# Veason-silverbullet/NNR

Measured on AMD Instinct MI355X. Metric: training impressions/sec on MIND-200k (CNE+SUE, bs=64), higher is better.
Workload: dtype f32

## Files before the change

### include/nnr_hip.h

```cpp
#ifndef NNR_HIP_H
#define NNR_HIP_H
#include <stdint.h>
#include <hip/hip_runtime_api.h>

#ifdef __cplusplus
extern "C" {
#endif

#define NNR_OK 0
#define NNR_ERR_ARG (-1)
#define NNR_ERR_LAUNCH (-2)
#define NNR_ERR_UNSUPPORTED (-3)

int nnr_version(void);

typedef struct nnr_gemm_args {
  const float* A;
  const float* B;
  float* C;
  int M, N, K;
  int lda, ldb, ldc;
  int trans_a, trans_b;
  const int* dyn_dev;
  int dyn_dim;
// ... 13 lines not shown
  int ldaux;
  const float* mul;
  int ldmul;
  const float* resid;
  int ldres;
  int accumulate;
  int atomic;
  const int* c_idx;
  int split_k;
  const float* rowdot_w;
  float* rowdot_out;
  int batch;
  long strideA, strideB, strideC, stride_aux, stride_res;
  int k_chunk;
  float* colsum_out;
  int tile;
  uint32_t drop_thresh;
  float drop_scale;
  int vec_epi;
  int sched;
  float* slab;
  long slab_floats;
  int slab_mode;
  const float* pre_add;
  int ldpre;
  int gate_bwd;
  const void* B3;
  long b3_stride;
  int ldb3;
} nnr_gemm_args;

int nnr_gemm_f32(const nnr_gemm_args* args, hipStream_t stream);
int nnr_split_bf16x3(const float* w, int rows, int cols, int ld, int ldo, void* out3, long img_stride, hipStream_t stream);

int nnr_seq_plan(uint8_t* mask, const int* ids, int n, int L, const int* perm_in, int* len_out, int* order, int* rank, int* slen,
                 int* bs, int* off, int* row_seq, int* tok, int* prev_f, int* prev_r, hipStream_t stream);

int nnr_seq_plan_pair(uint8_t* mask0, const int* ids0, int n0, uint8_t* mask1, const int* ids1, int n1, int L, const int* perm_in,
                      int* len_out, int* order, int* rank, int* slen, int* bs, int* off, int* row_seq, int* tok, int* prev_f,
                      int* prev_r, hipStream_t stream);

int nnr_cne_pair_map(const int* order_t, const int* order_c, int n0, int n, int* pm_t, int* pm_c, int* tmp, hipStream_t stream);

int nnr_mask_cover(const uint8_t* mask, int n, int L, uint8_t* cover, hipStream_t stream);
int nnr_seq_rowmap(const int* off, const int* rank, const int* len, int n, int L, int* rowmap, hipStream_t stream);

int nnr_lstm_dims(int H, int* UB, int* HP, int* NP);
int nnr_lstm_pack_weights(const float* w_ih_f, const float* w_hh_f, const float* b_ih_f, const float* b_hh_f, const float* w_ih_r,
                          const float* w_hh_r, const float* b_ih_r, const float* b_hh_r, int H, int E, float* w_ihp, float* b_p,
                          float* wf, float* wb, float* w_ihp_t, hipStream_t stream);
int nnr_lstm_unpack_grads(float* dw_ihp, float* db_p, float* dw_hhp, int H, int E, float* dw_ih_f, float* dw_hh_f,
                          float* db_ih_f, float* db_hh_f, float* dw_ih_r, float* dw_hh_r, float* db_ih_r, float* db_hh_r,
                          int accumulate , int zero_src, hipStream_t stream);
typedef struct nnr_lstm_problem {
  const int* bs; const int* off; const int* slen; const int* prev_f; const int* prev_r;
  int n, L;
  float* gates;
  float* cell;
  float* hout;
  float* cn;
  const float* wf;
  const float* wb;
  const float* dh;
  const float* dcn;
  unsigned* sync;
} nnr_lstm_problem;
// ... 202 lines not shown
```

### nnr_amd/_lib.py

```python
import ctypes as C
import os
import subprocess

_HERE = os.path.dirname(os.path.abspath(__file__))
LIB_PATH = os.environ.get('NNR_HIP_LIB') or os.path.join(_HERE, 'libnnr_hip.so')
_lib = None

vp, ci, cf, cu32, cl = C.c_void_p, C.c_int, C.c_float, C.c_uint32, C.c_long


class GemmArgs(C.Structure):
    _fields_ = [('A', vp), ('B', vp), ('C', vp), ('M', ci), ('N', ci), ('K', ci), ('lda', ci), ('ldb', ci), ('ldc', ci),
                ('trans_a', ci), ('trans_b', ci), ('dyn_dev', vp), ('dyn_dim', ci), ('a_idx', vp), ('b_idx', vp),
                ('drop_target', ci), ('drop_p', cf), ('drop_seed', cu32), ('drop_cols', ci), ('alpha', cf), ('bias', vp),
                ('rowvec', vp), ('ldrv', ci), ('rowvec_map', vp), ('act', ci), ('aux_out', vp), ('ldaux', ci), ('mul', vp),
                ('ldmul', ci), ('resid', vp), ('ldres', ci), ('accumulate', ci), ('atomic', ci), ('c_idx', vp),
                ('split_k', ci), ('rowdot_w', vp), ('rowdot_out', vp), ('batch', ci), ('strideA', cl), ('strideB', cl),
                ('strideC', cl), ('stride_aux', cl), ('stride_res', cl), ('k_chunk', ci), ('colsum_out', vp), ('tile', ci), ('drop_thresh', cu32),
                ('drop_scale', cf), ('vec_epi', ci), ('sched', ci), ('slab', vp), ('slab_floats', cl), ('slab_mode', ci), ('pre_add', vp), ('ldpre', ci), ('gate_bwd', ci), ('B3', vp), ('b3_stride', cl), ('ldb3', ci)]


class LstmProblem(C.Structure):
    _fields_ = [('bs', vp), ('off', vp), ('slen', vp), ('prev_f', vp), ('prev_r', vp), ('n', ci), ('L', ci), ('gates', vp),
                ('cell', vp), ('hout', vp), ('cn', vp), ('wf', vp), ('wb', vp), ('dh', vp), ('dcn', vp), ('sync', vp)]


class TransposeDesc(C.Structure):
    _fields_ = [('inp', vp), ('out', vp), ('rows', ci), ('cols', ci)]


class CorpusTables(C.Structure):
    _fields_ = [(k, vp) for k in ('news_category', 'news_subCategory', 'title_text', 'title_mask', 'title_entity', 'abstract_text',
                                  'abstract_mask', 'abstract_entity', 'beh_user', 'beh_history', 'beh_history_mask', 'beh_line',
                                  'graph_table', 'cmask_table', 'cidx_table')] + [(k, ci) for k in ('T', 'C', 'H', 'G', 'K1')]


class BatchOut(C.Structure):
    _fields_ = [(k, vp) for k in ('user_id', 'u_cat', 'u_sub', 'u_tt', 'u_tm', 'u_te', 'u_ct', 'u_cm', 'u_ce', 'u_hmask', 'u_graph',
                                  'u_cmask', 'u_cidx', 'n_cat', 'n_sub', 'n_tt', 'n_tm', 'n_te', 'n_ct', 'n_cm', 'n_ce')]


class PoolArgs(C.Structure):
    _fields_ = [('x', vp), ('ldx', ci), ('D', ci), ('n', ci), ('L', ci), ('packed', ci), ('off', vp), ('slen', vp),
                ('order', vp), ('mask', vp), ('mask_div', ci), ('score', vp), ('v', vp), ('ldv', ci), ('scale', cf),
                ('alpha', vp), ('out', vp), ('ldo', ci), ('add_in', vp), ('ldadd', ci), ('dout', vp), ('lddo', ci),
                ('dout2', vp), ('lddo2', ci), ('dx', vp), ('lddx', ci), ('dx_accumulate', ci), ('dscore', vp), ('dv', vp),
                ('lddv', ci), ('th', vp), ('ldth', ci), ('A', ci), ('w2', vp),
                ('alpha_b', vp), ('dout_b', vp), ('lddo_b', ci), ('dscore_b', vp), ('v_b', vp), ('ldv_b', ci), ('scale_b', cf)]


SYMBOLS = [
    'nnr_version', 'nnr_gemm_f32', 'nnr_split_bf16x3', 'nnr_seq_plan', 'nnr_seq_plan_pair', 'nnr_cne_pair_map', 'nnr_lstm_dims', 'nnr_lstm_pack_weights', 'nnr_lstm_unpack_grads',
    'nnr_lstm_fwd', 'nnr_lstm_bwd', 'nnr_lstm_sync_bytes', 'nnr_lstm_sync_diag_offset', 'nnr_lstm_set_timeout_counter', 'nnr_attn_pool_fwd', 'nnr_attn_pool_bwd', 'nnr_gate_bwd', 'nnr_packed_seq_sum',
    'nnr_tanh_score_bwd', 'nnr_slot_workspace_floats', 'nnr_colsum', 'nnr_rowdot', 'nnr_small_embed_fwd', 'nnr_small_embed_bwd', 'nnr_add', 'nnr_add_atomic', 'nnr_add2d', 'nnr_expand_rows_fwd', 'nnr_expand_rows_bwd', 'nnr_dropout',
    'nnr_layernorm_fwd', 'nnr_layernorm_bwd', 'nnr_relu_bwd', 'nnr_relu_drop_bwd', 'nnr_gcn_aggregate_fwd', 'nnr_gcn_aggregate_bwd', 'nnr_sue_x0_fwd', 'nnr_sue_x0_bwd', 'nnr_sue_slice_fwd', 'nnr_sue_slice_bwd',
    'nnr_sue_intra_fwd', 'nnr_sue_intra_bwd', 'nnr_logits_loss_fwd', 'nnr_logits_fwd', 'nnr_nls_loss', 'nnr_logits_bwd', 'nnr_sumsq', 'nnr_sumsq_part', 'nnr_clip_adam',
    'nnr_mhsa_fwd', 'nnr_mhsa_bwd', 'nnr_mhsa_fwd_packed', 'nnr_mhsa_bwd_packed', 'nnr_mhsa_pair_map', 'nnr_mhsa_fwd_paired', 'nnr_mhsa_bwd_paired', 'nnr_mask_cover', 'nnr_seq_rowmap', 'nnr_embed_gather', 'nnr_embed_scatter', 'nnr_embed_scatter_dyn', 'nnr_transpose2d', 'nnr_transpose_batch', 'nnr_corpus_batch', 'nnr_history_graph', 'nnr_rank_metrics',
    'nnr_dp_unique_id', 'nnr_dp_init', 'nnr_dp_allreduce', 'nnr_dp_broadcast', 'nnr_dp_destroy', 'nnr_dp_emulate_ranks', 'nnr_dp_busy',
    'nnr_fill_zero', 'nnr_copy_bytes', 'nnr_fill_column_u8', 'nnr_adam_skipped_steps', 'nnr_adam_skipped_peek', 'nnr_fusion_rows_fwd', 'nnr_fusion_rows_bwd', 'nnr_click_loss',
    'nnr_tape_create', 'nnr_tape_destroy', 'nnr_tape_fn_id', 'nnr_tape_fn_nargs', 'nnr_tape_call', 'nnr_tape_wait_stream', 'nnr_tape_event_record',
    'nnr_tape_event_wait', 'nnr_tape_segment', 'nnr_tape_patch', 'nnr_tape_finalize', 'nnr_tape_info', 'nnr_tape_replay', 'nnr_tape_prepare_timing', 'nnr_tape_timings', 'nnr_tape_timeline',
    'nnr_tape_last_error',
    'nnr_token_sort_workspace_bytes', 'nnr_token_sort', 'nnr_embed_scatter_sorted_workspace_floats', 'nnr_embed_scatter_sorted', 'nnr_fusion_rows_bwd_det',
    'nnr_rows_touch', 'nnr_rows_compact', 'nnr_rows_pack', 'nnr_rows_unpack',
    'nnr_cand_attn_ws_floats', 'nnr_cand_attn_fwd', 'nnr_cand_attn_bwd',
    'nnr_omap_ws_floats', 'nnr_omap_fwd', 'nnr_omap_bwd', 'nnr_omap_reg_fwd', 'nnr_omap_reg_bwd',
]


class NnrHipError(RuntimeError):
    pass


def build(force=False):
    if force:
        bdir = os.path.join(_HERE, 'csrc', 'build')
        if os.path.isdir(bdir):
            for f in os.listdir(bdir):
                os.remove(os.path.join(bdir, f))
    subprocess.check_call(['bash', os.path.join(_HERE, 'csrc', 'build.sh')])
    return LIB_PATH


def lib():
    global _lib
# ... 36 lines not shown
```

### nnr_amd/csrc/gemm.hip

```cpp
#include "common.h"
#include <stdlib.h>
#include <type_traits>

namespace {

template <int BK>
__device__ __forceinline__ int swz(int r16) {
  return BK == 16 ? ((4 - (r16 >> 2)) & 3) : BK == 32 ? ((r16 >> 1) & 7) : (r16 & 15);
}

template <int TM, int TN>
__device__ __forceinline__ void gemm_epilogue(const nnr_gemm_args& g, f32x4 (&acc)[TM][TN], float* lds, float* __restrict__ C, int m0,
                                              int n0, int M, int N, int z) {
  constexpr int BN = 16 * TN, E_LD = BN + 4;
  const int tid = threadIdx.x, lane = tid & 63, w = tid >> 6;
  const int r = lane & 15, kk = lane >> 4;
  const uint32_t dthr = g.drop_thresh;
  const float dscale = g.drop_scale;
  const bool use_atomic = !g.slab_mode && (g.atomic || g.split_k > 1 || g.k_chunk > 0);
  float* aux = g.aux_out;
  const float* res = g.resid;
  const float* mulp = g.mul;
  if (g.batch > 1 && g.split_k <= 1 && g.k_chunk <= 0) {
    if (aux) aux += (long)z * g.stride_aux;
// ... 809 lines not shown
  dim3 grid(nbm * nbn, 1, g.batch > 1 ? g.batch : 1), block(256);
  hipLaunchKernelGGL((gemm_nt_pipe_kernel<TM, TN, BK, NS, OCC, PRIO>), grid, block, 0, s, g);
  NNR_CHECK_LAUNCH();
  return NNR_OK;
}

static bool pipe_ok(const nnr_gemm_args& g) {
  auto al = [](const void* p) { return ((uintptr_t)p & 15) == 0; };
  return !g.trans_a && !g.trans_b && !g.b_idx && g.split_k <= 1 && g.k_chunk <= 0 && !g.rowdot_w && !g.colsum_out &&
         (g.drop_target == 0 || g.drop_target == 3 || g.drop_target == 4) && (g.K & 3) == 0 && (g.lda & 3) == 0 && (g.ldb & 3) == 0 &&
         al(g.A) && al(g.B) && (g.batch <= 1 || (((g.strideA | g.strideB) & 3) == 0)) && (g.dyn_dim == 0 || g.dyn_dim == 1);
}

typedef __bf16 bf16x8_t __attribute__((ext_vector_type(8)));
__device__ __forceinline__ void split3_bf16(float x, __bf16& h1, __bf16& h2, __bf16& h3) {
  const unsigned u = __builtin_bit_cast(unsigned, x), mag = u & 0x7fffffffu;
  const bool big = mag >= 0x7f7f8000u, nonfinite = mag >= 0x7f800000u;
  h1 = (__bf16)x;
  if (big) h1 = __builtin_bit_cast(__bf16, (unsigned short)((u >> 16) | (mag > 0x7f800000u ? 0x40u : 0u)));
  const float r1 = nonfinite ? 0.f : x - (float)h1;
  h2 = (__bf16)r1;
  const float r2 = r1 - (float)h2;
  h3 = (__bf16)r2;
}
__global__ void split_bf16x3_kernel(const float* __restrict__ w, int rows, int cols, int ld, int ldo, __bf16* __restrict__ out, long img_stride) {
  const long total = (long)rows * ldo;
  for (long i = blockIdx.x * (long)blockDim.x + threadIdx.x; i < total; i += (long)gridDim.x * blockDim.x) {
    const int r = (int)(i / ldo), c = (int)(i - (long)r * ldo);
    __bf16 a, b, d;
    split3_bf16(c < cols ? w[(long)r * ld + c] : 0.f, a, b, d);
    out[i] = a; out[img_stride + i] = b; out[2 * img_stride + i] = d;
  }
}
__device__ __forceinline__ int bx3_swzA(int r) { return ((r >> 1) & 1) | (((r >> 3) & 1) << 2); }
__device__ __forceinline__ int bx3_swzB(int r) { return (r >> 1) & 3; }

typedef unsigned u32x4_t __attribute__((ext_vector_type(4)));
__device__ __forceinline__ unsigned hi16_pair(float odd, float even) {
  return __builtin_amdgcn_perm(__float_as_uint(odd), __float_as_uint(even), 0x07060302u);
}
__device__ __forceinline__ void split3_trunc8(const f32x4& x0, const f32x4& x1, bf16x8_t& a1, bf16x8_t& a2, bf16x8_t& a3) {
  const float xs[8] = {x0[0], x0[1], x0[2], x0[3], x1[0], x1[1], x1[2], x1[3]};
  unsigned w1[4], w2[4], w3[4];
#pragma unroll
  for (int p = 0; p < 4; ++p) {
    const float xe = xs[2 * p], xo = xs[2 * p + 1];
    const unsigned h1 = hi16_pair(xo, xe);
    const float re = xe - __uint_as_float(h1 << 16), ro = xo - __uint_as_float(h1 & 0xffff0000u);
    const unsigned h2 = hi16_pair(ro, re);
    const float se = re - __uint_as_float(h2 << 16), so = ro - __uint_as_float(h2 & 0xffff0000u);
    w1[p] = h1; w2[p] = h2; w3[p] = hi16_pair(so, se);
  }
  a1 = __builtin_bit_cast(bf16x8_t, u32x4_t{w1[0], w1[1], w1[2], w1[3]});
  a2 = __builtin_bit_cast(bf16x8_t, u32x4_t{w2[0], w2[1], w2[2], w2[3]});
  a3 = __builtin_bit_cast(bf16x8_t, u32x4_t{w3[0], w3[1], w3[2], w3[3]});
}

template <int TM, int TN, int NS>
__global__ __launch_bounds__(256, (NS * (64 * TM * 128 + 3 * 16 * TN * 64) > 80 * 1024 ? 1 : 2)) void gemm_nt_bx3_kernel(nnr_gemm_args g) {
  constexpr int BM = 64 * TM, BN = 16 * TN, BK = 32;
  constexpr int A_BYTES = BM * BK * 4, B_IMG_BYTES = BN * BK * 2, STAGE_BYTES = A_BYTES + 3 * B_IMG_BYTES;
  constexpr int NIA = A_BYTES / 1024, NIB1 = B_IMG_BYTES / 1024;
  static_assert(A_BYTES % 1024 == 0 && B_IMG_BYTES % 1024 == 0 && NIA % 4 == 0, "tile shape");
  constexpr int E_LD = BN + 4;
  constexpr int LDS_BYTES = NS * STAGE_BYTES > 64 * E_LD * 4 ? NS * STAGE_BYTES : 64 * E_LD * 4;
  __shared__ __attribute__((aligned(1024))) unsigned char lds_raw[LDS_BYTES];
// ... 754 lines not shown
    case 2: return launch_cfg<1, 5, 16>(g, stream);
    case 3: return launch_cfg<2, 13, 16>(g, stream);
    case 4: return launch_cfg<2, 5, 16>(g, stream);
    case 5: return launch_cfg<2, 5, 32>(g, stream);
    case 6: return launch_cfg<1, 5, 64>(g, stream);
    case 9:  if (!pipe_ok(g) || g.a_idx) return NNR_ERR_ARG; return launch_pipe2<2, 5, 3, 2>(g, stream);
    case 15: if (!pipe_ok(g)) return NNR_ERR_ARG; return launch_pipe<2, 5, 16, 3, 4>(g, stream);
    case 16: if (!pipe_ok(g)) return NNR_ERR_ARG; return launch_pipe<2, 5, 16, 2, 5>(g, stream);
    case 20: if (!tn_pipe_ok(g)) return NNR_ERR_ARG; return launch_tn_pipe<2, 5, 3, 3>(g, stream);
    case 26: if (!tn_pipe_ok(g) || g.b_idx) return NNR_ERR_ARG; return launch_tn_pipe2<2, 5, 3, 3>(g, stream);
    case 27: if (!tn_pipe_ok(g)) return NNR_ERR_ARG; return launch_tn_pipe2<2, 13, 3, 2>(g, stream);
    case 30: if (!tn_pipe_ok(g)) return NNR_ERR_ARG; return launch_tn_pipe2<2, 10, 3, 2>(g, stream);
    case 50: if (!bx3_ok(g)) return NNR_ERR_ARG; return launch_bx3<2, 5, 2>(g, stream);
    case 51: if (!bx3_ok(g)) return NNR_ERR_ARG; return launch_bx3<1, 5, 2>(g, stream);
    case 32: if (!tn_pipe_ok(g)) return NNR_ERR_ARG; return launch_tn_pipe2<1, 13, 3, 2>(g, stream);
    case 7:
      if (g.pre_add || g.gate_bwd) return NNR_ERR_ARG;
      if (g.trans_a || g.a_idx || g.b_idx || g.c_idx || g.dyn_dev || g.split_k > 1 || g.k_chunk > 0 || g.rowdot_w || g.colsum_out || g.atomic ||
          (g.drop_target != 0 && g.drop_target != 3)) return NNR_ERR_ARG;
      return launch_skinny(g, stream);
    default: return NNR_ERR_ARG;
  }
}

extern "C" int nnr_split_bf16x3(const float* w, int rows, int cols, int ld, int ldo, void* out3, long img_stride, hipStream_t stream) {
  if (!w || !out3 || rows <= 0 || cols <= 0 || ld < cols || ldo < cols || (ldo & 7) || img_stride < (long)rows * ldo) return NNR_ERR_ARG;
  const long total = (long)rows * ldo;
  const int blocks = (int)((total + 255) / 256 > 1024 ? 1024 : (total + 255) / 256);
  hipLaunchKernelGGL(split_bf16x3_kernel, dim3(blocks), dim3(256), 0, stream, w, rows, cols, ld, ldo, reinterpret_cast<__bf16*>(out3), img_stride);
  NNR_CHECK_LAUNCH();
  return NNR_OK;
}

extern "C" int nnr_gemm_f32(const nnr_gemm_args* a, hipStream_t stream) {
  if (!a || !a->A || !a->B) return NNR_ERR_ARG;
  if (!a->C && !a->rowdot_out && !a->aux_out) return NNR_ERR_ARG;
  if (a->M <= 0 || a->N <= 0 || a->K <= 0) return NNR_OK;
  nnr_gemm_args g = *a;
  g.drop_thresh = nnr_drop_thresh(g.drop_target ? g.drop_p : 0.f);
  g.drop_scale = (g.drop_target && g.drop_p > 0.f) ? 1.f / (1.f - g.drop_p) : 1.f;
  if (g.drop_thresh == 0u) g.drop_target = 0;
  if (g.k_chunk > 0) { if ((g.k_chunk & 31) || g.batch > 1) return NNR_ERR_ARG; g.split_k = 2; }
  if (g.split_k > 1 && (g.bias || g.rowvec || g.act || g.aux_out || g.mul || g.resid || g.batch > 1 || g.rowdot_w))
    return NNR_ERR_ARG;
  if ((g.a_idx && g.trans_a) || (g.b_idx && !g.trans_b)) return NNR_ERR_ARG;
  if (g.colsum_out && !g.trans_a) return NNR_ERR_ARG;
  if ((g.dyn_dim != 0) != (g.dyn_dev != nullptr)) return NNR_ERR_ARG;
  {
    auto ok = [](const void* p, int ld) { return p == nullptr || ((((uintptr_t)p) & 15) == 0 && (ld & 3) == 0); };
    const bool strides = g.batch <= 1 || (((g.strideC | g.stride_aux | g.stride_res) & 3) == 0);
    g.vec_epi = (!g.c_idx && !g.atomic && g.split_k <= 1 && !g.rowdot_w && (g.N & 3) == 0 && ok(g.C, g.ldc) && ok(g.bias, 0) &&
                 ok(g.rowvec, g.ldrv) && ok(g.aux_out, g.ldaux) && ok(g.mul, g.ldmul) && ok(g.resid, g.ldres) && strides &&
                 (g.drop_target != 3 || (g.drop_cols & 3) == 0)) ? 1 : 0;
  }
  if (g.pre_add || g.gate_bwd) {
    auto al = [](const void* p, int ld) { return p != nullptr && (((uintptr_t)p) & 15) == 0 && (ld & 3) == 0; };
    if (!g.vec_epi || g.split_k > 1 || g.k_chunk > 0 || g.batch > 1 || (g.pre_add && !al(g.pre_add, g.ldpre))) return NNR_ERR_ARG;
    if (g.gate_bwd && (!g.C || !g.aux_out || !g.mul || !g.resid || g.bias || g.rowvec || g.act || g.drop_target || g.accumulate || g.rowdot_w)) return NNR_ERR_ARG;
  }
  float* slab_C = nullptr;
  float* slab_cs = nullptr;
  int slab_ldc = 0;
  if (g.slab != nullptr) {
    if (!(g.trans_a && g.trans_b) || g.split_k <= 1 || g.k_chunk > 0 || g.c_idx || (g.N & 3) || (((uintptr_t)g.slab) & 15) || !g.C || g.accumulate == 2 ||
        g.slab_floats < (long)g.split_k * ((long)g.M * g.N + g.M))
      return NNR_ERR_ARG;
// ... 38 lines not shown
```

### nnr_amd/csrc/tape.hip

```cpp
#include <cstring>
#include <string>
#include <tuple>
#include <utility>
#include <vector>
#include "common.h"

namespace {

typedef int (*thunk_t)(const uint64_t* slots, hipStream_t stream);

template <typename T> inline T slot_as(const uint64_t* s) { T v; std::memcpy(&v, s, sizeof(T)); return v; }

template <auto Fn> struct Thunk;
template <typename... P, int (*Fn)(P...)> struct Thunk<Fn> {
  static constexpr int nargs = (int)sizeof...(P) - 1;
  template <size_t... I> static int apply(const uint64_t* s, hipStream_t st, std::index_sequence<I...>) {
    using Tup = std::tuple<P...>;
    static_assert(std::is_same<std::tuple_element_t<sizeof...(P) - 1, Tup>, hipStream_t>::value, "entry point must end with hipStream_t");
    return Fn(slot_as<std::tuple_element_t<I, Tup>>(s + I)..., st);
  }
  static int call(const uint64_t* s, hipStream_t st) { return apply(s, st, std::make_index_sequence<sizeof...(P) - 1>{}); }
};

struct Entry { const char* name; thunk_t thunk; int nargs; };
#define R(fn) { #fn, &Thunk<&fn>::call, Thunk<&fn>::nargs }
const Entry REGISTRY[] = {
  R(nnr_gemm_f32), R(nnr_seq_plan), R(nnr_seq_plan_pair), R(nnr_cne_pair_map), R(nnr_lstm_pack_weights), R(nnr_lstm_unpack_grads),
  R(nnr_lstm_fwd), R(nnr_lstm_bwd), R(nnr_attn_pool_fwd), R(nnr_attn_pool_bwd), R(nnr_gate_bwd), R(nnr_packed_seq_sum),
  R(nnr_tanh_score_bwd), R(nnr_colsum), R(nnr_rowdot), R(nnr_small_embed_fwd), R(nnr_small_embed_bwd), R(nnr_embed_gather),
  R(nnr_embed_scatter), R(nnr_embed_scatter_dyn), R(nnr_transpose2d), R(nnr_transpose_batch), R(nnr_add), R(nnr_add_atomic), R(nnr_add2d), R(nnr_expand_rows_fwd), R(nnr_expand_rows_bwd),
  R(nnr_dropout), R(nnr_relu_bwd), R(nnr_gcn_aggregate_fwd), R(nnr_gcn_aggregate_bwd), R(nnr_relu_drop_bwd), R(nnr_mhsa_fwd), R(nnr_mhsa_bwd),
  R(nnr_sue_x0_fwd), R(nnr_sue_x0_bwd), R(nnr_sue_slice_fwd), R(nnr_sue_slice_bwd), R(nnr_sue_intra_fwd), R(nnr_sue_intra_bwd),
  R(nnr_corpus_batch), R(nnr_history_graph), R(nnr_logits_loss_fwd), R(nnr_logits_fwd), R(nnr_nls_loss), R(nnr_logits_bwd),
  R(nnr_layernorm_fwd), R(nnr_layernorm_bwd), R(nnr_sumsq), R(nnr_sumsq_part), R(nnr_clip_adam), R(nnr_dp_allreduce), R(nnr_dp_broadcast), R(nnr_dp_busy), R(nnr_split_bf16x3), R(nnr_mhsa_fwd_packed), R(nnr_mhsa_bwd_packed), R(nnr_mhsa_pair_map), R(nnr_mhsa_fwd_paired), R(nnr_mhsa_bwd_paired), R(nnr_mask_cover), R(nnr_seq_rowmap),
  R(nnr_fill_zero), R(nnr_copy_bytes), R(nnr_fill_column_u8), R(nnr_fusion_rows_fwd), R(nnr_fusion_rows_bwd), R(nnr_click_loss), R(nnr_rank_metrics),
  R(nnr_token_sort), R(nnr_embed_scatter_sorted), R(nnr_fusion_rows_bwd_det),
  R(nnr_rows_touch), R(nnr_rows_compact), R(nnr_rows_pack), R(nnr_rows_unpack),
  R(nnr_cand_attn_fwd), R(nnr_cand_attn_bwd),
  R(nnr_omap_fwd), R(nnr_omap_bwd), R(nnr_omap_reg_fwd), R(nnr_omap_reg_bwd),
};
#undef R
constexpr int NREG = (int)(sizeof(REGISTRY) / sizeof(REGISTRY[0]));

enum { OP_CALL = 0, OP_RECORD = 1, OP_WAIT = 2 };
struct Op { int kind, a, b; };
struct Call { int fn, stream, nslots, tag; size_t slot_off; };
struct BlobRef { size_t slot; size_t blob_off; };
struct Patch { size_t byte_off; int kind; int width; int64_t addend; };
constexpr int MAX_TIMING_SETS = 64;

}

struct nnr_tape {
  std::vector<uint64_t> arena;
  std::vector<Call> calls;
  std::vector<Op> ops;
  std::vector<size_t> seg_begin;
  std::vector<hipStream_t> streams;
  std::vector<hipEvent_t> events;
  std::vector<uint64_t> event_keys;
  std::vector<BlobRef> blob_refs;
  std::vector<Patch> patches;
  std::vector<std::vector<hipEvent_t>> tset;
  int ntagged = 0;
  bool final = false;
  int last_rc = 0, last_failed_call = -1;
};
// ... 245 lines not shown
```

### nnr_amd/news_encoders.py

```python
import math
import os
import pickle

import torch
import torch.nn as nn

from . import ops
from .layers import Attention, ScaledDotProduct_CandidateAttention, MultiHeadAttention, Conv1D, LSTMParams, grad_of

_SITE = dict(title=1, content=2, cat=3, sub=4)
_DP_TABLE_FIRST = int(os.environ.get('NNR_DP_TABLE_FIRST', '0'))


def _dp_world():
    import torch.distributed as dist
    return dist.get_world_size() if dist.is_initialized() else 1


class NewsEncoder(nn.Module):

    def __init__(self, config, word_table=None):
        super().__init__()
        self.word_embedding_dim = config.word_embedding_dim
        self.word_embedding = nn.Embedding(num_embeddings=config.vocabulary_size, embedding_dim=self.word_embedding_dim)
# ... 116 lines not shown

    def __enter__(self):
        if self.side is not None:
            self.ctx = torch.cuda.stream(self.side)
            self.ctx.__enter__()

    def __exit__(self, *a):
        if self.side is not None:
            self.ctx.__exit__(*a)


def _fork_join(n_calls, dev, phase):
    if n_calls == 1:
        return [phase(0, True)]
    main = torch.cuda.current_stream(dev)
    side = _side_stream(dev)
    side.wait_stream(main)
    with torch.cuda.stream(side):
        first = phase(0, False)
    rest = [phase(i, True) for i in range(1, n_calls)]
    main.wait_stream(side)
    return [first] + rest


def cne_forward_many(mod, calls):
    H, E = mod.hidden_dim, mod.word_embedding_dim
    dev = (calls[0][0][0] if isinstance(calls[0][0], tuple) else calls[0][0]).device
    if len(calls) > 1:
        ops.lstm_pack(mod.title_lstm, H, E)
        ops.lstm_pack(mod.content_lstm, H, E)
    else:
        ops.lstm_prefetch(dev, (mod.title_lstm, mod.content_lstm), H, E)
    if mod.training:
        ops.bx3_prefetch(dev)
    pre = _fork_join(len(calls), dev, lambda i, on_main: _cne_fwd_pre(mod, *calls[i], par=on_main))
    items = [sv['streams'][1] for sv in pre] + [sv['streams'][0] for sv in pre]
    for i in range(0, len(items), 4):
        ops.lstm_fwd(items[i:i + 4], H)
    return _fork_join(len(calls), dev, lambda i, on_main: _cne_fwd_post(mod, pre[i], on_main))


def _torch_tie_perm(masks):
    perms, lens = [], []
    base = 0
    for m in masks:
        l = (m.sum(dim=1).long() + (~m[:, 0]).long()).cpu()
        q = torch.sort(l, descending=True)[1]
        perms.append(q + base)
        lens.append(l[q])
        base += m.shape[0]
    if len(perms) == 1:
        return perms[0].to(torch.int32)
    q, l = torch.cat(perms), torch.cat(lens)
    return q[torch.sort(l, descending=True, stable=True)[1]].to(torch.int32)


def _cne_fwd_pre(mod, title_text, title_mask, content_text, content_mask, category, subCategory, par=False, partner=None):
    union = isinstance(title_text, tuple)
    if union:
        B, N = title_text[0].shape[:2]
        n0 = B * N
        n = n0 + B * title_text[1].shape[1]
        dev = title_text[0].device
    else:
        B, N = title_text.shape[:2]
        n = n0 = B * N
        dev = title_text.device
# ... 455 lines not shown
```

### nnr_amd/ops.py

```python
import ctypes as C
import math
import os
import weakref

import torch

from . import _lib as L
from . import profile as _prof
from . import tape as _tape

ACT_NONE, ACT_RELU, ACT_TANH, ACT_SIGMOID = 0, 1, 2, 3
K_CHUNK = 1024


class _NoSpan:
    def __enter__(self):
        return self

    def __exit__(self, *a):
        return False


_NOSPAN = _NoSpan()

# ... 143 lines not shown


def leaf_deferred(dev, rows, fn, *tensors):
    if _DEFER.get('off') or max(rows, STEP_ROWS[0]) < LEAF_MIN_ROWS:
        fn()
        return
    leaf, main = leaf_stream(dev), torch.cuda.current_stream(dev)
    leaf.wait_stream(main)
    _DEFER['keep'].extend(tensors)
    _DEFER['calls'] += 1
    with torch.cuda.stream(leaf):
        fn()
    if _DEFER.get('manual'):
        return
    if not _DEFER['queued']:
        _DEFER['queued'] = True
        try:
            torch.autograd.Variable._execution_engine.queue_callback(lambda: join_extra_streams(dev))
        except RuntimeError:
            join_extra_streams(dev)


def tape_keep(*tensors):
    t = _tape.ACTIVE[0]
    if t is not None:
        t.keep.extend(x for x in tensors if x is not None)


PARAM_EPOCH = [0]
_DERIVED = {}
_OWNED = {}
_DERIVED_SWEEP = 256
_WT_DESCS = [None, None]


class _Derived:
    __slots__ = ('ref', 'ptr', 'spec', 'out', 'bufs', 'prefetch', 'stamp', 'gen', 'event', 'stream', 'served')


def is_weight(t):
    return isinstance(t, torch.nn.Parameter) or id(t) in _OWNED


def _drop(key):
    for b in _DERIVED.pop(key).bufs:
        _OWNED.pop(id(b), None)


def _derived(kind, src, spec, make, prefetch):
    key = (kind, id(src))
    ptr = src.data_ptr() if torch.is_tensor(src) else None
    e = _DERIVED.get(key)
    if e is not None and e.ref() is src and e.ptr == ptr and e.spec == spec:
        return e
    if e is not None:
        _drop(key)
    if len(_DERIVED) > _DERIVED_SWEEP:
        for k in [k for k, v in _DERIVED.items() if v.ref() is None]:
            _drop(k)
    e = _DERIVED[key] = _Derived()
    e.ref, e.ptr, e.spec, e.prefetch = weakref.ref(src), ptr, spec, prefetch
    e.out = make()
    e.bufs = (e.out,) if torch.is_tensor(e.out) else e.out.bufs
    e.stamp, e.gen, e.event, e.stream, e.served = None, 0, None, None, False
    for b in e.bufs:
        _OWNED[id(b)] = e
    return e


def _stamp(sources):
    t = _tape.ACTIVE[0]
    s = [PARAM_EPOCH[0], None if t is None else weakref.ref(t)]
    for x in sources:
        o = _OWNED.get(id(x))
        s.append(o.gen if o is not None else (x.data_ptr(), x._version))
    return tuple(s)


def _refreshed(jobs, stream):
    ev = torch.cuda.Event()
    ev.record()
    for e, stamp in jobs:
        e.stamp, e.gen, e.event, e.stream = stamp, e.gen + 1, ev, stream


def _serve(e, sources, fill):
    e.served = True
    tape_keep(*e.bufs)
    stamp, cur = _stamp(sources), _s().value
    if e.stamp != stamp:
        fill()
        _refreshed([(e, stamp)], cur)
    elif e.stream != cur:
        torch.cuda.current_stream(e.bufs[0].device).wait_event(e.event)


def _stale(kind):
    jobs = []
    for (k, _), e in _DERIVED.items():
        src = e.ref() if k == kind and e.prefetch and e.served else None
        if src is not None and src.data_ptr() == e.ptr:
            stamp = _stamp((src,))
            if e.stamp != stamp:
                jobs.append((e, src, stamp))
    return jobs


def _on_leaf(dev, jobs, launch):
    leaf = leaf_stream(dev)
    leaf.wait_stream(torch.cuda.current_stream(dev))
    with torch.cuda.stream(leaf):
        launch()
        _refreshed([(e, stamp) for e, _, stamp in jobs], _s().value)
    for e, _, _ in jobs:
        e.served = False


def wt(w):
    rows, cols = w.shape
    e = _derived('wt', w, (rows, cols), lambda: torch.empty((cols, rows), device=w.device, dtype=torch.float32), isinstance(w, torch.nn.Parameter))
    _serve(e, (w,), lambda: transpose2d(w, e.out, rows, cols))
    return e.out


def wt_prefetch(dev):
    if torch.cuda.is_current_stream_capturing():
        return
    jobs = _stale('wt')
    if not jobs:
        return
    descs = tuple((w.data_ptr(), e.out.data_ptr(), w.shape[0], w.shape[1]) for e, w, _ in jobs)
    if _WT_DESCS[0] != descs:
        arr = (L.TransposeDesc * len(descs))()
        for d, (src, out, rows, cols) in zip(arr, descs):
            d.inp, d.out, d.rows, d.cols = src, out, rows, cols
        _WT_DESCS[:] = [descs, torch.frombuffer(bytearray(bytes(arr)), dtype=torch.uint8).to(dev)]
    table = _WT_DESCS[1]
    tape_keep(table, *[e.out for e, _, _ in jobs])
    _on_leaf(dev, jobs, lambda: L.check(L.lib().nnr_transpose_batch(_p(table), len(descs), _s()), 'nnr_transpose_batch'))


def _pack_entry(lstm, p, H, E):
    return _derived('lstm', lstm, (H, E), lambda: LstmPacked(p, H, E, fill=False), False)


def lstm_pack(lstm, H, E):
    p = lstm.param_list()
    e = _pack_entry(lstm, p, H, E)
    _serve(e, p, lambda: e.out.pack(p))
    return e.out


def lstm_prefetch(dev, lstms, H, E):
    jobs = []
    for lstm in lstms:
        p = lstm.param_list()
        e = _pack_entry(lstm, p, H, E)
        stamp = _stamp(p)
        if e.stamp != stamp:
            jobs.append((e, p, stamp))

    def launch():
        for e, p, _ in jobs:
            tape_keep(*e.bufs)
            e.out.pack(p)
    if jobs:
        _on_leaf(dev, jobs, launch)


def tn_tile(M, N, K, gather=False):
    if K >= 2048 and M >= 512 and N >= 512 and not gather and not ((M & 3) or (N & 3)):
        return 26, 128, 80, 2048
# ... 12 lines not shown

def split_for(m, n, k, tile_m=64, tile_n=80, target_blocks=2048, kmin=256):
    tiles = max(1, ((m + tile_m - 1) // tile_m) * ((n + tile_n - 1) // tile_n))
    if k <= 640:
        return 1
    return int(max(1, min((k + kmin - 1) // kmin, (target_blocks + tiles - 1) // tiles)))


BX3 = [os.environ.get('NNR_BX3', '1') == '1']
_BX3_MIN_ROWS = 2048
_BX3_TILE = 50
_BX3_CLASSES = {'dx', 'sue', 'proj', 'gate'}


def bx3_class(N, K):
    if K >= 1024:
        return 'dx'
    if K >= 800:
        return 'sue'
    if N >= 1024:
        return 'proj'
    return 'gate'


BX3_SEEN = {}


def _split_bf16x3(B, N, K, ldb, img):
    ldo = img.shape[2]
    L.check(L.lib().nnr_split_bf16x3(_p(B), N, K, ldb, ldo, _p(img), C.c_long(N * ldo), _s()), 'nnr_split_bf16x3')


def bx3_prefetch(dev):
    if not BX3[0] or torch.cuda.is_current_stream_capturing():
        return
    jobs = _stale('bx3')

    def launch():
        for e, B, _ in jobs:
            tape_keep(e.out, B)
            _split_bf16x3(B, *e.spec, e.out)
    if jobs:
        _on_leaf(dev, jobs, launch)


def bx3_images(B, N, K, ldb):
    ldo = (K + 7) // 8 * 8
    owner = _OWNED.get(id(B))
    e = _derived('bx3', B, (N, K, ldb), lambda: torch.empty((3, N, ldo), device=B.device, dtype=torch.int16),
                 isinstance(B, torch.nn.Parameter) or (owner is not None and owner.prefetch))
    _serve(e, (B,), lambda: _split_bf16x3(B, N, K, ldb, e.out))
    return e.out, N * ldo, ldo


def _bx3_wanted(A, B, M, N, K, lda, ldb, trans_a, trans_b, a_idx, b_idx, c_idx, split_k, k_chunk, rowdot_w, colsum_out, atomic, batch, dyn_dim, drop):
    return (not trans_a and not trans_b and a_idx is None and b_idx is None and split_k <= 1 and k_chunk <= 0 and rowdot_w is None
            and colsum_out is None and batch <= 1 and dyn_dim in (0, 1) and M >= _BX3_MIN_ROWS and K >= 64 and N * K <= (1 << 22)
            and (K | lda | ldb) & 3 == 0 and (A.data_ptr() | B.data_ptr()) & 15 == 0 and (drop is None or drop[0] in (3, 4) or drop[1] <= 0.0))


def gemm(A, B, C_=None, *, M, N, K, lda, ldb, ldc=0, trans_a=False, trans_b=False, dyn=None, dyn_dim=0, a_idx=None, b_idx=None,
         drop=None, alpha=1.0, bias=None, rowvec=None, ldrv=0, rowvec_map=None, act=0, aux_out=None, ldaux=0, mul=None, ldmul=0,
         resid=None, ldres=0, accumulate=False, atomic=False, c_idx=None, split_k=1, rowdot_w=None, rowdot_out=None, batch=1,
         strideA=0, strideB=0, strideC=0, stride_aux=0, stride_res=0, tile=0, colsum_out=None, k_chunk=0, flop_scale=1.0, slab=None,
         pre_add=None, ldpre=0, gate_bwd=False, b3=None):
    g = L.GemmArgs()
    g.A, g.B = A.data_ptr(), B.data_ptr()
    if C_ is not None:
        g.C = C_.data_ptr()
    g.M, g.N, g.K, g.lda, g.ldb, g.ldc, g.alpha = M, N, K, lda, ldb, ldc, alpha
    if trans_a:
        g.trans_a = 1
    if trans_b:
        g.trans_b = 1
    if dyn is not None:
        g.dyn_dev, g.dyn_dim = dyn.data_ptr(), dyn_dim
    if a_idx is not None:
        g.a_idx = a_idx.data_ptr()
    if b_idx is not None:
        g.b_idx = b_idx.data_ptr()
    if drop is not None and drop[1] > 0.0:
        g.drop_target, g.drop_p, g.drop_seed, g.drop_cols = drop[0], float(drop[1]), int(drop[2]) & 0xFFFFFFFF, int(drop[3])
    if bias is not None:
# ... 826 lines not shown
```

### nnr_amd/step.py

```python
import contextlib

import torch

from . import ops
from .news_encoders import cne_forward_many, cne_backward_many

_BX3_MIN_SEQS = 1408


def kind(model):
    from . import news_encoders as NE, user_encoders as UE
    if model.click_predictor != 'dot_product' or not model.training:
        return None
    if type(model.news_encoder) is NE.CNE and type(model.user_encoder) is UE.SUE and model.news_encoder.tie_order == 'stable' and NE._CNE_UNION:
        return 'cne_sue'
    if type(model.news_encoder) is NE.MHSA and type(model.user_encoder) is UE.MHSA:
        return 'mhsa'
    return None


def step_sequences(batch):
    return int(batch[15].shape[0]) * (int(batch[15].shape[1]) + int(batch[3].shape[1]))


# ... 150 lines not shown
                _mhsa_news_backward(ne, nodes_c, dcand)
                _mhsa_news_backward(ne, nodes_h, dhist.reshape(B, Hn, D))
        finally:
            ops._DEFER['manual'] = False
        ops.join_extra_streams()
    return logits, loss


def forward_backward(trainer, batch):
    model = trainer.model
    if kind(model) == 'mhsa':
        with matrix_path(model, batch):
            return forward_backward_mhsa(trainer, batch)
    ne, ue = model.news_encoder, model.user_encoder
    (user_ID, user_category, user_subCategory, user_title_text, user_title_mask, user_title_entity, user_content_text, user_content_mask,
     user_content_entity, user_history_mask, user_history_graph, user_history_category_mask, user_history_category_indices, news_category,
     news_subCategory, news_title_text, news_title_mask, news_title_entity, news_content_text, news_content_mask, news_content_entity) = batch
    dev = news_title_text.device
    f32 = dict(device=dev, dtype=torch.float32)
    ops._DEFER['step_joins'] = True
    try:
        with matrix_path(model, batch):
            return _forward_backward_cne_sue(trainer, model, ne, ue, batch, dev, f32)
    finally:
        ops._DEFER['step_joins'] = False


def _forward_backward_cne_sue(trainer, model, ne, ue, batch, dev, f32):
    (user_ID, user_category, user_subCategory, user_title_text, user_title_mask, user_title_entity, user_content_text, user_content_mask,
     user_content_entity, user_history_mask, user_history_graph, user_history_category_mask, user_history_category_indices, news_category,
     news_subCategory, news_title_text, news_title_mask, news_title_entity, news_content_text, news_content_mask, news_content_entity) = batch
    with torch.no_grad():
        ops.STEP_ROWS[0] = 0
        ops.wt_prefetch(dev)
        cand = (news_title_text, news_title_mask, news_content_text, news_content_mask, news_category, news_subCategory)
        hist = (user_title_text, user_title_mask, user_content_text, user_content_mask, user_category, user_subCategory)
        ((rep_c, rep_h), sv), = cne_forward_many(ne, [tuple(zip(cand, hist))])
        B, N, D = rep_c.shape
        n0 = B * N
        n = n0 + rep_h.shape[0] * rep_h.shape[1]
        from .user_encoders import sue_forward, sue_backward
        assert user_history_graph.is_contiguous() and user_history_category_indices.is_contiguous()
        user, ssv = sue_forward(ue, rep_h, rep_c, user_history_graph, user_history_category_mask, user_history_category_indices)
        logits = torch.empty((B, N), **f32)
        loss = torch.empty((), **f32)
        drep = torch.empty((n, D), **f32)
        duser = torch.empty((B, N, D), **f32)
        trainer.wait_grad_zeroed()
        ops.click_loss(user, rep_c, B, N, D, logits, loss, None, duser, drep[:n0], torch.empty(B, **f32))
        sue_backward(ue, ssv, duser, dhist_out=drep[n0:].view(B, -1, D), dcand_accum=drep[:n0])
        cne_backward_many(ne, [(sv, drep)])
        ops.join_extra_streams()
    return logits, loss
```

Before: 6712.

## Batch bf16x3 weight splits into one descriptor-driven kernel with weight-transpose prefetch

Replaces the per-weight bf16x3 split launches with a single batched kernel driven by a device descriptor table, and merges it with the weight-transpose prefetch into one weights_prefetch call. When the split source is a pending transposed copy, it reads the original weight with a shared-memory transpose tile instead of waiting for the copy. The goal is fewer kernel launches and less host-side Python overhead per step, and removing the dependency on the transpose copy. It adds staleness-stamp logic for pending entries, which could mis-track cache freshness.

```diff
diff --git a/include/nnr_hip.h b/include/nnr_hip.h
--- a/include/nnr_hip.h
+++ b/include/nnr_hip.h
@@ -69,6 +69,10 @@
 
 int nnr_gemm_f32(const nnr_gemm_args* args, hipStream_t stream);
 int nnr_split_bf16x3(const float* w, int rows, int cols, int ld, int ldo, void* out3, long img_stride, hipStream_t stream);
+#define NNR_SPLIT_ROWS 8
+#define NNR_SPLIT_ROWS_T 32
+typedef struct nnr_split_desc { const float* w; void* out3; long img_stride; int rows, cols, ld, ldo, transposed, blk0; } nnr_split_desc;
+int nnr_split_bf16x3_batch(const nnr_split_desc* descs_dev, int count, hipStream_t stream);
 
 int nnr_seq_plan(uint8_t* mask, const int* ids, int n, int L, const int* perm_in, int* len_out, int* order, int* rank, int* slen,
                  int* bs, int* off, int* row_seq, int* tok, int* prev_f, int* prev_r, hipStream_t stream);
diff --git a/nnr_amd/_lib.py b/nnr_amd/_lib.py
--- a/nnr_amd/_lib.py
+++ b/nnr_amd/_lib.py
@@ -29,6 +29,11 @@
     _fields_ = [('inp', vp), ('out', vp), ('rows', ci), ('cols', ci)]
 
 
+class SplitDesc(C.Structure):
+    _fields_ = [('w', vp), ('out3', vp), ('img_stride', cl), ('rows', ci), ('cols', ci), ('ld', ci), ('ldo', ci), ('transposed', ci), ('blk0', ci)]
+    ROWS, ROWS_T = 8, 32
+
+
 class CorpusTables(C.Structure):
     _fields_ = [(k, vp) for k in ('news_category', 'news_subCategory', 'title_text', 'title_mask', 'title_entity', 'abstract_text',
                                   'abstract_mask', 'abstract_entity', 'beh_user', 'beh_history', 'beh_history_mask', 'beh_line',
@@ -50,7 +55,7 @@
 
 
 SYMBOLS = [
-    'nnr_version', 'nnr_gemm_f32', 'nnr_split_bf16x3', 'nnr_seq_plan', 'nnr_seq_plan_pair', 'nnr_cne_pair_map', 'nnr_lstm_dims', 'nnr_lstm_pack_weights', 'nnr_lstm_unpack_grads',
+    'nnr_version', 'nnr_gemm_f32', 'nnr_split_bf16x3', 'nnr_split_bf16x3_batch', 'nnr_seq_plan', 'nnr_seq_plan_pair', 'nnr_cne_pair_map', 'nnr_lstm_dims', 'nnr_lstm_pack_weights', 'nnr_lstm_unpack_grads',
     'nnr_lstm_fwd', 'nnr_lstm_bwd', 'nnr_lstm_sync_bytes', 'nnr_lstm_sync_diag_offset', 'nnr_lstm_set_timeout_counter', 'nnr_attn_pool_fwd', 'nnr_attn_pool_bwd', 'nnr_gate_bwd', 'nnr_packed_seq_sum',
     'nnr_tanh_score_bwd', 'nnr_slot_workspace_floats', 'nnr_colsum', 'nnr_rowdot', 'nnr_small_embed_fwd', 'nnr_small_embed_bwd', 'nnr_add', 'nnr_add_atomic', 'nnr_add2d', 'nnr_expand_rows_fwd', 'nnr_expand_rows_bwd', 'nnr_dropout',
     'nnr_layernorm_fwd', 'nnr_layernorm_bwd', 'nnr_relu_bwd', 'nnr_relu_drop_bwd', 'nnr_gcn_aggregate_fwd', 'nnr_gcn_aggregate_bwd', 'nnr_sue_x0_fwd', 'nnr_sue_x0_bwd', 'nnr_sue_slice_fwd', 'nnr_sue_slice_bwd',
diff --git a/nnr_amd/csrc/gemm.hip b/nnr_amd/csrc/gemm.hip
--- a/nnr_amd/csrc/gemm.hip
+++ b/nnr_amd/csrc/gemm.hip
@@ -865,6 +865,72 @@
     out[i] = a; out[img_stride + i] = b; out[2 * img_stride + i] = d;
   }
 }
+constexpr int SPLIT_ROWS = NNR_SPLIT_ROWS, SPLIT_ROWS_T = NNR_SPLIT_ROWS_T, SPLIT_TC = 128;
+static_assert(SPLIT_ROWS_T == 32, "the transposed-source tile is 32 rows x SPLIT_TC columns on 32 x 8 threads");
+__global__ __launch_bounds__(256) void split_bf16x3_batch_kernel(const nnr_split_desc* __restrict__ descs, int count) {
+  __shared__ float tile[SPLIT_TC][33];
+  const int tid = threadIdx.x;
+  const nnr_split_desc last = descs[count - 1];
+  const int total = last.blk0 + (last.rows + (last.transposed ? SPLIT_ROWS_T : SPLIT_ROWS) - 1) / (last.transposed ? SPLIT_ROWS_T : SPLIT_ROWS);
+  for (int item = blockIdx.x; item < total; item += gridDim.x) {
+    int lo = 0, hi = count - 1;
+    while (lo < hi) {
+      const int mid = (lo + hi + 1) >> 1;
+      if (descs[mid].blk0 <= item) lo = mid; else hi = mid - 1;
+    }
+    const nnr_split_desc d = descs[lo];
+    const int rb = d.transposed ? SPLIT_ROWS_T : SPLIT_ROWS;
+    const long r0 = (long)(item - d.blk0) * rb;
+    if (item < d.blk0 || r0 >= d.rows || d.cols > d.ldo) continue;
+    __bf16* __restrict__ out = reinterpret_cast<__bf16*>(d.out3);
+    if (!d.transposed) {
+      const int n = (int)(d.rows - r0 < rb ? d.rows - r0 : rb) * d.ldo;
+      const long o0 = r0 * d.ldo;
+      for (int base = 0; base < n; base += 4 * 256) {
+        float v[4];
+#pragma unroll
+        for (int u = 0; u < 4; ++u) {
+          const int i = base + u * 256 + tid, r = i / d.ldo, c = i - r * d.ldo;
+          v[u] = (i < n && c < d.cols) ? d.w[(r0 + r) * d.ld + c] : 0.f;
+        }
+#pragma unroll
+        for (int u = 0; u < 4; ++u) {
+          const int i = base + u * 256 + tid;
+          if (i < n) {
+            __bf16 a, b, e;
+            split3_bf16(v[u], a, b, e);
+            out[o0 + i] = a; out[d.img_stride + o0 + i] = b; out[2 * d.img_stride + o0 + i] = e;
+          }
+        }
+      }
+    } else {
+      const int tx = tid & 31, ty = tid >> 5;
+      for (int c0 = 0; c0 < d.ldo; c0 += SPLIT_TC) {
+        const long r = r0 + tx;
+#pragma unroll
+        for (int j = ty; j < SPLIT_TC; j += 8) {
+          const int c = c0 + j;
+          tile[j][tx] = (r < d.rows && c < d.cols) ? d.w[(long)c * d.ld + r] : 0.f;
+        }
+        __syncthreads();
+        for (int j = ty; j < 32; j += 8) {
+          const long rr = r0 + j;
+#pragma unroll
+          for (int q = 0; q < SPLIT_TC; q += 32) {
+            const int c = c0 + q + tx;
+            if (rr < d.rows && c < d.ldo) {
+              __bf16 a, b, e;
+              split3_bf16(tile[q + tx][j], a, b, e);
+              const long o = rr * d.ldo + c;
+              out[o] = a; out[d.img_stride + o] = b; out[2 * d.img_stride + o] = e;
+            }
+          }
+        }
+        __syncthreads();
+      }
+    }
+  }
+}
 __device__ __forceinline__ int bx3_swzA(int r) { return ((r >> 1) & 1) | (((r >> 3) & 1) << 2); }
 __device__ __forceinline__ int bx3_swzB(int r) { return (r >> 1) & 3; }
 
@@ -1685,6 +1751,14 @@
   return NNR_OK;
 }
 
+extern "C" int nnr_split_bf16x3_batch(const nnr_split_desc* descs_dev, int count, hipStream_t stream) {
+  if (count <= 0) return NNR_OK;
+  if (!descs_dev) return NNR_ERR_ARG;
+  hipLaunchKernelGGL(split_bf16x3_batch_kernel, dim3(4096), dim3(256), 0, stream, descs_dev, count);
+  NNR_CHECK_LAUNCH();
+  return NNR_OK;
+}
+
 extern "C" int nnr_gemm_f32(const nnr_gemm_args* a, hipStream_t stream) {
   if (!a || !a->A || !a->B) return NNR_ERR_ARG;
   if (!a->C && !a->rowdot_out && !a->aux_out) return NNR_ERR_ARG;
diff --git a/nnr_amd/csrc/tape.hip b/nnr_amd/csrc/tape.hip
--- a/nnr_amd/csrc/tape.hip
+++ b/nnr_amd/csrc/tape.hip
@@ -32,7 +32,7 @@
   R(nnr_dropout), R(nnr_relu_bwd), R(nnr_gcn_aggregate_fwd), R(nnr_gcn_aggregate_bwd), R(nnr_relu_drop_bwd), R(nnr_mhsa_fwd), R(nnr_mhsa_bwd),
   R(nnr_sue_x0_fwd), R(nnr_sue_x0_bwd), R(nnr_sue_slice_fwd), R(nnr_sue_slice_bwd), R(nnr_sue_intra_fwd), R(nnr_sue_intra_bwd),
   R(nnr_corpus_batch), R(nnr_history_graph), R(nnr_logits_loss_fwd), R(nnr_logits_fwd), R(nnr_nls_loss), R(nnr_logits_bwd),
-  R(nnr_layernorm_fwd), R(nnr_layernorm_bwd), R(nnr_sumsq), R(nnr_sumsq_part), R(nnr_clip_adam), R(nnr_dp_allreduce), R(nnr_dp_broadcast), R(nnr_dp_busy), R(nnr_split_bf16x3), R(nnr_mhsa_fwd_packed), R(nnr_mhsa_bwd_packed), R(nnr_mhsa_pair_map), R(nnr_mhsa_fwd_paired), R(nnr_mhsa_bwd_paired), R(nnr_mask_cover), R(nnr_seq_rowmap),
+  R(nnr_layernorm_fwd), R(nnr_layernorm_bwd), R(nnr_sumsq), R(nnr_sumsq_part), R(nnr_clip_adam), R(nnr_dp_allreduce), R(nnr_dp_broadcast), R(nnr_dp_busy), R(nnr_split_bf16x3), R(nnr_split_bf16x3_batch), R(nnr_mhsa_fwd_packed), R(nnr_mhsa_bwd_packed), R(nnr_mhsa_pair_map), R(nnr_mhsa_fwd_paired), R(nnr_mhsa_bwd_paired), R(nnr_mask_cover), R(nnr_seq_rowmap),
   R(nnr_fill_zero), R(nnr_copy_bytes), R(nnr_fill_column_u8), R(nnr_fusion_rows_fwd), R(nnr_fusion_rows_bwd), R(nnr_click_loss), R(nnr_rank_metrics),
   R(nnr_token_sort), R(nnr_embed_scatter_sorted), R(nnr_fusion_rows_bwd_det),
   R(nnr_rows_touch), R(nnr_rows_compact), R(nnr_rows_pack), R(nnr_rows_unpack),
diff --git a/nnr_amd/news_encoders.py b/nnr_amd/news_encoders.py
--- a/nnr_amd/news_encoders.py
+++ b/nnr_amd/news_encoders.py
@@ -172,7 +172,7 @@
     else:
         ops.lstm_prefetch(dev, (mod.title_lstm, mod.content_lstm), H, E)
     if mod.training:
-        ops.bx3_prefetch(dev)
+        ops.weights_prefetch(dev)
     pre = _fork_join(len(calls), dev, lambda i, on_main: _cne_fwd_pre(mod, *calls[i], par=on_main))
     items = [sv['streams'][1] for sv in pre] + [sv['streams'][0] for sv in pre]
     for i in range(0, len(items), 4):
diff --git a/nnr_amd/ops.py b/nnr_amd/ops.py
--- a/nnr_amd/ops.py
+++ b/nnr_amd/ops.py
@@ -199,10 +199,11 @@
 _OWNED = {}
 _DERIVED_SWEEP = 256
 _WT_DESCS = [None, None]
+_BX3_DESCS = [None, None]
 
 
 class _Derived:
-    __slots__ = ('ref', 'ptr', 'spec', 'out', 'bufs', 'prefetch', 'stamp', 'gen', 'event', 'stream', 'served')
+    __slots__ = ('kind', 'ref', 'ptr', 'spec', 'out', 'bufs', 'prefetch', 'stamp', 'gen', 'event', 'stream', 'served')
 
 
 def is_weight(t):
@@ -226,7 +227,7 @@
         for k in [k for k, v in _DERIVED.items() if v.ref() is None]:
             _drop(k)
     e = _DERIVED[key] = _Derived()
-    e.ref, e.ptr, e.spec, e.prefetch = weakref.ref(src), ptr, spec, prefetch
+    e.kind, e.ref, e.ptr, e.spec, e.prefetch = kind, weakref.ref(src), ptr, spec, prefetch
     e.out = make()
     e.bufs = (e.out,) if torch.is_tensor(e.out) else e.out.bufs
     e.stamp, e.gen, e.event, e.stream, e.served = None, 0, None, None, False
@@ -235,12 +236,12 @@
     return e
 
 
-def _stamp(sources):
+def _stamp(sources, pending=()):
     t = _tape.ACTIVE[0]
     s = [PARAM_EPOCH[0], None if t is None else weakref.ref(t)]
     for x in sources:
         o = _OWNED.get(id(x))
-        s.append(o.gen if o is not None else (x.data_ptr(), x._version))
+        s.append(o.gen + (o in pending) if o is not None else (x.data_ptr(), x._version))
     return tuple(s)
 
 
@@ -262,12 +263,12 @@
         torch.cuda.current_stream(e.bufs[0].device).wait_event(e.event)
 
 
-def _stale(kind):
+def _stale(kind, pending=()):
     jobs = []
     for (k, _), e in _DERIVED.items():
         src = e.ref() if k == kind and e.prefetch and e.served else None
         if src is not None and src.data_ptr() == e.ptr:
-            stamp = _stamp((src,))
+            stamp = _stamp((src,), pending)
             if e.stamp != stamp:
                 jobs.append((e, src, stamp))
     return jobs
@@ -291,20 +292,58 @@
 
 
 def wt_prefetch(dev):
+    weights_prefetch(dev, images=False)
+
+
+def _table(cache, descs, struct, fill, dev):
+    if cache[0] != descs:
+        arr = (struct * len(descs))()
+        for d, v in zip(arr, descs):
+            fill(d, v)
+        cache[:] = [descs, torch.frombuffer(bytearray(bytes(arr)), dtype=torch.uint8).to(dev)]
+    return cache[1]
+
+
+def _wt_desc(d, v):
+    d.inp, d.out, d.rows, d.cols = v
+
+
+def _bx3_desc(d, v):
+    d.w, d.out3, d.img_stride, d.rows, d.cols, d.ld, d.ldo, d.transposed, d.blk0 = v
+
+
+def weights_prefetch(dev, copies=True, images=True):
     if torch.cuda.is_current_stream_capturing():
         return
-    jobs = _stale('wt')
-    if not jobs:
-        return
-    descs = tuple((w.data_ptr(), e.out.data_ptr(), w.shape[0], w.shape[1]) for e, w, _ in jobs)
-    if _WT_DESCS[0] != descs:
-        arr = (L.TransposeDesc * len(descs))()
-        for d, (src, out, rows, cols) in zip(arr, descs):
-            d.inp, d.out, d.rows, d.cols = src, out, rows, cols
-        _WT_DESCS[:] = [descs, torch.frombuffer(bytearray(bytes(arr)), dtype=torch.uint8).to(dev)]
-    table = _WT_DESCS[1]
-    tape_keep(table, *[e.out for e, _, _ in jobs])
-    _on_leaf(dev, jobs, lambda: L.check(L.lib().nnr_transpose_batch(_p(table), len(descs), _s()), 'nnr_transpose_batch'))
+    wt_jobs = _stale('wt') if copies else []
+    pending = {e for e, _, _ in wt_jobs}
+    bx_jobs, bx_descs, blk = [], [], 0
+    for e, B, stamp in (_stale('bx3', pending) if images and BX3[0] else []):
+        N, K, ldb = e.spec
+        o = _OWNED.get(id(B))
+        w = o.ref() if o is not None and o.kind == 'wt' else None
+        if w is not None and w.data_ptr() == o.ptr and o.spec == (K, N) and ldb == K:
+            src, ld, tr = w, N, 1
+        elif o in pending:
+            continue
+        else:
+            src, ld, tr = B, ldb, 0
+        ldo = e.out.shape[2]
+        bx_jobs.append((e, B, stamp))
+        bx_descs.append((src.data_ptr(), e.out.data_ptr(), N * ldo, N, K, ld, ldo, tr, blk))
+        blk += -(-N // (L.SplitDesc.ROWS_T if tr else L.SplitDesc.ROWS))
+        tape_keep(e.out, B, src)
+    launches = []
+    if bx_jobs:
+        table = _table(_BX3_DESCS, tuple(bx_descs), L.SplitDesc, _bx3_desc, dev)
+        tape_keep(table)
+        launches.append(lambda: L.check(L.lib().nnr_split_bf16x3_batch(_p(table), len(bx_descs), _s()), 'nnr_split_bf16x3_batch'))
+    if wt_jobs:
+        wt_table = _table(_WT_DESCS, tuple((w.data_ptr(), e.out.data_ptr(), w.shape[0], w.shape[1]) for e, w, _ in wt_jobs), L.TransposeDesc, _wt_desc, dev)
+        tape_keep(wt_table, *[e.out for e, _, _ in wt_jobs])
+        launches.append(lambda: L.check(L.lib().nnr_transpose_batch(_p(wt_table), len(wt_jobs), _s()), 'nnr_transpose_batch'))
+    if launches:
+        _on_leaf(dev, wt_jobs + bx_jobs, lambda: [f() for f in launches])
 
 
 def _pack_entry(lstm, p, H, E):
@@ -383,23 +422,14 @@
 
 
 def bx3_prefetch(dev):
-    if not BX3[0] or torch.cuda.is_current_stream_capturing():
-        return
-    jobs = _stale('bx3')
-
-    def launch():
-        for e, B, _ in jobs:
-            tape_keep(e.out, B)
-            _split_bf16x3(B, *e.spec, e.out)
-    if jobs:
-        _on_leaf(dev, jobs, launch)
+    weights_prefetch(dev, copies=False)
 
 
 def bx3_images(B, N, K, ldb):
     ldo = (K + 7) // 8 * 8
     owner = _OWNED.get(id(B))
     e = _derived('bx3', B, (N, K, ldb), lambda: torch.empty((3, N, ldo), device=B.device, dtype=torch.int16),
-                 isinstance(B, torch.nn.Parameter) or (owner is not None and owner.prefetch))
+                 isinstance(B, torch.nn.Parameter) or (owner is not None and (owner.prefetch or owner.kind == 'lstm')))
     _serve(e, (B,), lambda: _split_bf16x3(B, N, K, ldb, e.out))
     return e.out, N * ldo, ldo
 
diff --git a/nnr_amd/step.py b/nnr_amd/step.py
--- a/nnr_amd/step.py
+++ b/nnr_amd/step.py
@@ -206,7 +206,6 @@
      news_subCategory, news_title_text, news_title_mask, news_title_entity, news_content_text, news_content_mask, news_content_entity) = batch
     with torch.no_grad():
         ops.STEP_ROWS[0] = 0
-        ops.wt_prefetch(dev)
         cand = (news_title_text, news_title_mask, news_content_text, news_content_mask, news_category, news_subCategory)
         hist = (user_title_text, user_title_mask, user_content_text, user_content_mask, user_category, user_subCategory)
         ((rep_c, rep_h), sv), = cne_forward_many(ne, [tuple(zip(cand, hist))])
```

After: 6713, median of 4. About the same (+0.0%).
